# SysCV/LiDAR_snow_sim

Measured on AMD Instinct MI355X. Metric: augmented points/s/GPU (64x2048 sweep, 2.5 mm/h); HBM roofline % -- value: rows resident in HBM when the clock starts (device-resident API: augment_batch on CUDA tensors); with H2D of the rows and D2H of the results inside the clock: value_pcie_inclusive, higher is better.
Workload: dtype f64

## Files before the change

lidar_snow_sim_amd/csrc/sg_few.h:

```cpp
#pragma once
#include "sg_beam.h"

template <int N>
struct SgFew {
    double amp[N], rho[N];
    int k0[N], k1[N];
    double tamp, d;
    int tk0, tk1;
    int S;
};

template <typename T, int N>
__device__ __forceinline__ int sg_few_prep(double d, double theta_c, int L, const double (&a1_in)[N], const double (&a2_in)[N], const double (&rho)[N],
                                           int channel, const SgLasers *__restrict__ las, double beam_div_deg, SgFew<N> &p, SgBeamOut &out)
{
    constexpr bool F32 = SgReal<T>::is_f32;
    static_assert(N >= 1 && N <= 3, "an owner must stay below eight slots (2 N + 1 <= 7)");
    const int max_i = las->max_i[channel];
    double a1[N], a2[N];
    double theta_r, theta_l;
    sg_beam_limits(theta_c, beam_div_deg, theta_r, theta_l);
    double ra = theta_r, la = theta_l;
    const bool wrap = ra > la;
    if (wrap) ra = ra - SG_TWO_PI;
#pragma unroll
    for (int j = 0; j < N; ++j) {
        a1[j] = a1_in[j]; a2[j] = a2_in[j];
        if (wrap && j < L && a1[j] > a2[j]) a1[j] = a1[j] - SG_TWO_PI;
    }
    const double delta = beam_div_deg * (SG_PI / 180.0);
    double e_min = ra < la ? ra : la, e_max = ra < la ? la : ra;
#pragma unroll
    for (int j = 0; j < N; ++j) {
        if (j < L) {
            const double lo = a1[j], hi = a2[j];
            if (lo < e_min) e_min = lo;
            if (hi < e_min) e_min = hi;
            if (lo > e_max) e_max = lo;
            if (hi > e_max) e_max = hi;
        }
    }
    double R[N], tsum = -0.0;
    bool has[N];
#pragma unroll
    for (int j = 0; j < N; ++j) { R[j] = 0.0; has[j] = false; }
    for (double e = e_min; e < e_max;) {
        int own = -1;
        double nxt = e_max;
#pragma unroll
        for (int j = 0; j < N; ++j) {
            if (j < L) {
                if (own < 0 && a1[j] <= e && e < a2[j]) own = j;
                if (a1[j] > e && a1[j] < nxt) nxt = a1[j];
                if (a2[j] > e && a2[j] < nxt) nxt = a2[j];
            }
        }
        if (ra > e && ra < nxt) nxt = ra;
        if (la > e && la < nxt) nxt = la;
        const double w = nxt - e;
        if (own < 0) tsum += w;
#pragma unroll
        for (int j = 0; j < N; ++j)
            if (own == j) { R[j] = has[j] ? R[j] + w : w; has[j] = true; }
        e = nxt;
    }
    const double c_tau = 299792458.0 * 1e-8;
    const double beta_0 = 1 * 1e-6 / SG_PI;
    const double i_snow = 0.9 * max_i;
    const double ca_p0 = i_snow / beta_0;
#pragma unroll
    for (int t = 0; t < N; ++t) { p.amp[t] = 0.0; p.rho[t] = 0.0; p.k0[t] = 0; p.k1[t] = 0; }
    int S = 0;
#pragma unroll
    for (int j = 0; j < N; ++j) {
        if (j < L && has[j]) {
            const double ratio = sg_clip01((0.0 + R[j]) / delta);
            const double r = rho[j];
            int k0 = (int)ceil(r * 10);
            int k1 = (int)(floor((r + c_tau) * 10) + 1);
            const double amp = (((ca_p0 * beta_0) * ratio) * sg_xsi(r)) / (r * r);
            if (k1 > SG_RBINS) { out.range_error = 1; k1 = SG_RBINS; }
            if (k0 < 0) k0 = 0;
#pragma unroll
            for (int t = 0; t <= j; ++t)
                if (t == S) { p.amp[t] = amp; p.rho[t] = r; p.k0[t] = k0; p.k1[t] = k1; }
            ++S;
        }
    }
    p.S = S;
    p.d = d;
    p.tamp = 0.0; p.tk0 = 0; p.tk1 = 0;
    if (S == 0) return 0;
    const double ratio_t = sg_clip01((0.0 + tsum) / delta);
    if constexpr (F32) {
        const float r = (float)(T)d;
        p.tk0 = (int)ceilf(r * 10.0f);
        float ee = r + (float)c_tau;
        ee = ee * 10.0f;
        ee = floorf(ee) + 1.0f;
        p.tk1 = (int)ee;
        const float r2 = r * r;
        p.tamp = (((ca_p0 * beta_0) * ratio_t) * sg_xsi(r)) / (double)r2;
    } else {
        p.tk0 = (int)ceil(d * 10);
        p.tk1 = (int)(floor((d + c_tau) * 10) + 1);
        p.tamp = (((ca_p0 * beta_0) * ratio_t) * sg_xsi(d)) / (d * d);
    }
    if (p.tk1 > SG_RBINS) { out.range_error = 1; p.tk1 = SG_RBINS; }
    if (p.tk0 < 0) p.tk0 = 0;
    out.n_flakes = S;
    out.has_power = 1;
    return S;
}

template <int N, int TT>
__device__ __forceinline__ void sg_few_zone(const SgFew<N> &p, double best, int &ka, int &kb)
{
    constexpr bool TARGET = TT == N;
    const double c_tau = 299792458.0 * 1e-8;
    const double step = (120 + c_tau) / (SG_RBINS - 1);
    ka = 0; kb = -1;
    double A, r;
    int k0, k1;
    if constexpr (TARGET) { A = p.tamp; r = p.d; k0 = p.tk0; k1 = p.tk1; }
    else { if (TT >= p.S) return; A = p.amp[TT]; r = p.rho[TT]; k0 = p.k0[TT]; k1 = p.k1[TT]; }
    if (!(A > 0.0)) return;
    double oth = 0.0;
    int lo_trim = k0, hi_trim = k1;
    auto visit = [&](double Aj, int q0, int q1, bool first) {
        if (Aj > A || (Aj == A && first)) {
            if (q0 <= k0) { if (q1 > lo_trim) lo_trim = q1; }
            else if (q1 >= k1) { if (q0 < hi_trim) hi_trim = q0; }
        } else oth += Aj;
    };
    bool go = true;
#pragma unroll
    for (int j = N - 1; j >= 0; --j) {
        if (j < TT && j < p.S && go) {
            if (p.k1[j] <= k0) go = false;
            else visit(p.amp[j], p.k0[j], p.k1[j], true);
        }
    }
    if constexpr (!TARGET) {
        go = true;
#pragma unroll
        for (int j = 0; j < N; ++j) {
            if (j > TT && j < p.S && go) {
                if (p.k0[j] >= k1) go = false;
                else visit(p.amp[j], p.k0[j], p.k1[j], false);
            }
        }
        if (go && !(p.tk0 >= k1)) visit(p.tamp, p.tk0, p.tk1, false);
    }
    double amax = p.tamp;
#pragma unroll
    for (int j = 0; j < N; ++j) if (j < p.S) amax = fmax(amax, p.amp[j]);
    const double need = fmax(best, 0.9966 * amax);
    if ((A + oth) * (1.0 + 1e-9) < need) return;
    const double q = (need * (1.0 - 1e-9) - oth * (1.0 + 1e-9)) / A;
    ka = k0; kb = k1 - 1;
    if (q >= 0.5) {
        const double om = q < 1.0 ? 1.0 - q : 0.0;
        const double dl = (double)sqrtf((float)(1.26 * om)) * (1.0 + 1e-6) + 1e-6;
        const double Rc = r + c_tau / 2;
        const double D = dl * (c_tau / SG_PI) + 0.006;
        const int za = (int)ceil((Rc - D) * (1.0 / step)), zb = (int)floor((Rc + D) * (1.0 / step));
        if (za > ka) ka = za;
        if (zb < kb) kb = zb;
    }
    if (lo_trim > ka) ka = lo_trim;
    if (hi_trim - 1 < kb) kb = hi_trim - 1;
}

template <bool EXACT, int N>
__device__ __forceinline__ double sg_few_bin(const double (&amp)[N], const double (&rho)[N], const int (&k0)[N], const int (&k1)[N],
                                             double tamp, double d, int tk0, int tk1, int k, const double *__restrict__ rgrid)
{
    const double Rk = EXACT ? rgrid[k < SG_RBINS ? k : SG_RBINS - 1] : sg_range_bin(k);
    double sm = 0.0;
#pragma unroll
    for (int t = 0; t < N; ++t)
        if (k >= k0[t] && k < k1[t]) sm += sg_power_term<EXACT>(amp[t], Rk, rho[t]);
    if (k >= tk0 && k < tk1) sm += sg_power_term<EXACT>(tamp, Rk, d);
    return sm;
}
```

lidar_snow_sim_amd/csrc/snowgpu_kernels.hip:

```cpp
#include <hip/hip_runtime.h>
#include <algorithm>
#include "sg_beam.h"
#include "sg_few.h"
#include "sg_queue.h"
#include "sg_kutil.h"
#include "sg_launch.h"

#ifndef SG_NB4
#define SG_NB4 4
#endif
#ifndef SG_KP_WIN
#define SG_KP_WIN 3
#endif
#ifndef SG_FP_WAVES
#define SG_FP_WAVES 6
#endif
#ifndef SG_FP_WAVES_SEG
#define SG_FP_WAVES_SEG 7
#endif
#ifndef SG_NB_TIERS
#define SG_NB_TIERS 4
#endif
#ifndef SG_KP_THREE_MAX
#define SG_KP_THREE_MAX 16
// ... 390 lines not shown
        if ((threadIdx.x & 63) == 63 && total > 0) b = atomicAdd(counter, total);
        return __shfl(b, 63) + inc - n;
    };
    int base = reserve(n_items, a.pw_count);
    if (a.pw_items1) {
        int base1 = reserve(n_one, a.pw_count + 1);
        for (int k = 0; k < nf; k += lanes)
            a.pw_items1[base1++] = make_int2((int)(q_base + k), (nf - k < lanes ? nf - k : lanes) | (f1 << 10));
    } else {
        for (int k = 0; k < nf; k += lanes)
            a.pw_items[base++] = make_int2((int)(q_base + k), (nf - k < lanes ? nf - k : lanes) | (f1 << 10));
    }
    for (int k = 0; k < nb; k += lanes_back)
        a.pw_items[base++] = make_int2((int)(q_base + q_size - nb + k), (nb - k < lanes_back ? nb - k : lanes_back) | (f1 << 10));
}

__global__ __launch_bounds__(256) void k_tier_gather(SgBeamArgs a, int n_regions_ub)
{
    const int r = blockIdx.x * 4 + (int)(threadIdx.x >> 6), lane = (int)(threadIdx.x & 63);
    if (blockIdx.x == 0 && threadIdx.x < SG_MAX_CLASSES) a.status[2 + threadIdx.x] = a.tier_info[threadIdx.x];
    if (blockIdx.x == 0 && threadIdx.x < SG_MAX_CLASSES && a.tier_hint) a.tier_hint[threadIdx.x] = a.tier_info[threadIdx.x];
    if (blockIdx.x == 0 && threadIdx.x == 0 && a.tier_hint) a.tier_hint[SG_MAX_CLASSES] = (int32_t)((a.n_total >> 10) + 1);
    int q_size = 0, f1 = 0;
    int64_t q_base = 0;
    if (!sg_region(a, r, n_regions_ub, q_base, q_size, f1)) return;
    for (int k = 0; k < a.n_cls; ++k) {
        const int c = a.tn[(int64_t)r * SG_MAX_CLASSES + k];
        if (c == 0) continue;
        const int32_t *src = a.tier_sparse + (int64_t)k * a.tier_stride + q_base;
        int32_t *dst = a.tier_list + (int64_t)k * a.tier_stride + a.tbase[(int64_t)r * SG_MAX_CLASSES + k];
        for (int i = lane; i < c; i += 64) dst[i] = src[i];
    }
}

__device__ __forceinline__ const SgEntry *sg_dq_entries(const SgBeamArgs &a, int f, int ch)
{
    return a.frame_tables[(int64_t)f * a.las->n + ch].entries;
}

template <typename T, int LMAX, int BLOCK, bool LISTQ>
__device__ __forceinline__ void sg_kp_item(const SgBeamArgs &a, char *smem, const int ov_list, const int64_t work_off,
                                           const int start, const int cnt, const int item_f)
{
    constexpr int LANES = BLOCK < 64 ? BLOCK : 64;
    constexpr int WIN = BLOCK < 64 ? 1 : SG_KP_WIN;
    constexpr int P = SG_QPLANES(LMAX);
    double *s_a1 = (double *)smem;
    constexpr bool THREE = SG_KP_THREE_MAX > 0 && LMAX <= SG_KP_THREE_MAX && LMAX >= SG_KP_THREE_MIN;
    double *s_a2 = s_a1 + (LMAX + 1) * BLOCK;
    double *s_rho = s_a2 + (LMAX + 1) * BLOCK;
    double *s_ratio = THREE ? s_rho : s_rho + (LMAX + 1) * BLOCK;
    double *s_work = THREE ? s_a2 : s_ratio;
    const int tid = threadIdx.x, lane = tid & 63;
    const int ltid = BLOCK < 64 ? lane : tid;
    const double *planes = a.tq;
    const uint16_t *scs = LISTQ ? a.tq_sc : a.dq_sc;
    static_assert(WIN <= 4, "the window's permutation passes through one 64-double row segment of the wave");
    uint16_t *s_perm = (uint16_t *)(s_ratio + (BLOCK < 64 ? 0 : (tid & ~63)));
    int perm[WIN];
    const bool sorted = WIN > 1 && cnt > LANES;
    if constexpr (WIN > 1) {
        if (sorted) {
            int key[WIN], rank[WIN];
            int64_t at[WIN];
            unsigned scw[WIN];
#pragma unroll
            for (int r = 0; r < WIN; ++r) { const int idx = r * 64 + lane; at[r] = (int64_t)start + (idx < cnt ? idx : 0); }
            if (LISTQ && ov_list) {
#pragma unroll
                for (int r = 0; r < WIN; ++r) at[r] = (int64_t)a.tier_list[work_off + at[r]];
#pragma unroll
                for (int r = 0; r < WIN; ++r) scw[r] = (unsigned)a.ov_sc[at[r]];
            } else {
#pragma unroll
                for (int r = 0; r < WIN; ++r) scw[r] = (unsigned)scs[at[r]];
            }
#pragma unroll
            for (int r = 0; r < WIN; ++r) {
                const int idx = r * 64 + lane;
                key[r] = 255;
                if (idx < cnt) key[r] = scw[r] == 0xffffu ? 254 : (int)(scw[r] & 255u);
                rank[r] = 0;
            }
            int base = 0;
            auto place = [&](int c) {
#pragma unroll
                for (int r = 0; r < WIN; ++r) {
                    const unsigned long long m = __ballot(key[r] == c);
                    if (key[r] == c) rank[r] = base + (int)__popcll(m & sg_lanemask_lt());
                    base += (int)__popcll(m);
                }
            };
            for (int c = 0; c <= LMAX; ++c) place(c);
            place(254); place(255);
#pragma unroll
            for (int r = 0; r < WIN; ++r) s_perm[rank[r]] = (uint16_t)(r * 64 + lane);
            asm volatile("s_waitcnt lgkmcnt(0)" ::: "memory");
#pragma unroll
            for (int r = 0; r < WIN; ++r) perm[r] = s_perm[r * 64 + lane];
            asm volatile("s_waitcnt lgkmcnt(0)" ::: "memory");
        }
    }
    const int rounds = (cnt + LANES - 1) / LANES;
    for (int r = 0; r < rounds; ++r) {
        const int idx = r * LANES + lane;
        const bool in = lane < LANES && idx < cnt;
        int pos = idx;
        if constexpr (WIN > 1) {
            if (sorted) {
#pragma unroll
                for (int q = 0; q < WIN; ++q) if (q == r) pos = perm[q];
            }
        }
        const int64_t slot = (int64_t)start + pos;
        unsigned sc = 0xffffu;
        int32_t g = 0;
        double d = 0.0, tc = 0.0, f_rho = 0.0;
        [[maybe_unused]] double f_a1 = 0.0, f_a2 = 0.0;
        [[maybe_unused]] const double *qb = planes;
        [[maybe_unused]] int qs = 64;
        constexpr int NW = LMAX <= 4 ? LMAX : 1;
        [[maybe_unused]] uint32_t hw[NW];
#pragma unroll
        for (int j = 0; j < NW; ++j) hw[j] = 0u;
        if (in) {
            if constexpr (LISTQ) {
                g = a.tier_list[work_off + slot];
                if (ov_list) { qb = a.ov + (size_t)g * SG_OV_STRIDE; qs = 1; sc = a.ov_sc[g]; }
                else { qb = planes + sg_qaddr<P>(slot, 0); sc = scs[slot]; }
                d = qb[0];
                tc = qb[qs];
                f_a1 = qb[2 * qs]; f_a2 = qb[3 * qs]; f_rho = qb[4 * qs];
            } else {
                g = a.dq_g[slot];
                sc = scs[slot];
                sg_dq_load_header<T>(a.dq, slot, LMAX, d, tc);
#pragma unroll
                for (int j = 0; j < NW; ++j) hw[j] = sg_dq_load_word<T>(a.dq, slot, LMAX, j);
            }
        }
        const bool live = in && sc != 0xffffu;
        const int L = (int)(sc & 255u), ch = (int)(sc >> 8);
        int f = 0;
        SgBeamOut o;
        o.overflow = 0; o.range_error = 0; o.diff2 = 0.0; o.has_power = 0; o.n_flakes = 0; o.n_hits = 0; o.label = 0; o.new_i = 0; o.k_best = 0;
        constexpr int NB = LMAX <= 4 ? SG_NB4 : SG_NB_TIERS;
        int S = 0, nw = 0, k_best = 0;
        double best = 0.0;
        if (live) {
            f = item_f >= 0 ? item_f : sg_frame_of(a, g);
            unsigned long long ord = 0xfedcba9876543210ull;
            [[maybe_unused]] const SgEntry *ent = nullptr;
            if constexpr (LISTQ) {
                s_a1[ltid] = f_a1; s_a2[ltid] = f_a2; s_rho[ltid] = f_rho;
                if constexpr (THREE) ord = 0;
                for (int h0 = 1; h0 < L; h0 += 8) {
                    double xa[8], xb[8], xr[8];
#pragma unroll
                    for (int c = 0; c < 8; ++c) {
                        const int h = h0 + c < L ? h0 + c : 0;
                        xa[c] = qb[(2 + 3 * h) * qs]; xb[c] = qb[(3 + 3 * h) * qs]; xr[c] = qb[(4 + 3 * h) * qs];
                    }
#pragma unroll
                    for (int c = 0; c < 8; ++c)
                        if (h0 + c < L) { s_a1[(h0 + c) * BLOCK + ltid] = xa[c]; s_a2[(h0 + c) * BLOCK + ltid] = xb[c]; s_rho[(h0 + c) * BLOCK + ltid] = xr[c]; }
                }
                for (int h = 1; h < L; ++h) {
                    const double x1 = s_a1[h * BLOCK + ltid], x2 = s_a2[h * BLOCK + ltid], r = s_rho[h * BLOCK + ltid];
                    int q = h;
                    while (q > 0 && (s_rho[(q - 1) * BLOCK + ltid] > r ||
                                     (s_rho[(q - 1) * BLOCK + ltid] == r && ov_list &&
                                      (s_a1[(q - 1) * BLOCK + ltid] > x1 || (s_a1[(q - 1) * BLOCK + ltid] == x1 && s_a2[(q - 1) * BLOCK + ltid] > x2))))) {
                        s_rho[q * BLOCK + ltid] = s_rho[(q - 1) * BLOCK + ltid]; s_a1[q * BLOCK + ltid] = s_a1[(q - 1) * BLOCK + ltid];
                        s_a2[q * BLOCK + ltid] = s_a2[(q - 1) * BLOCK + ltid];
                        --q;
                    }
                    if (q != h) { s_rho[q * BLOCK + ltid] = r; s_a1[q * BLOCK + ltid] = x1; s_a2[q * BLOCK + ltid] = x2; }
                    if constexpr (THREE) {
                        const unsigned long long low = (1ull << (4 * q)) - 1ull;
                        ord = (ord & low) | ((unsigned long long)h << (4 * q)) | ((ord & ~low) << 4);
                    }
                }
            } else {
                ent = sg_dq_entries(a, f, ch);
                double th_r, th_l;
                sg_beam_limits(tc, a.beam_div_deg, th_r, th_l);
                if constexpr (LMAX <= 4) {
                    double xa[LMAX], xb[LMAX], xr[LMAX];
                    sg_dq_resolve_all<LMAX>(hw, L, ent, th_r, th_l, xa, xb, xr);
                    f_rho = xr[0];
#pragma unroll
                    for (int j = 0; j < LMAX; ++j)
                        if (j < L) {
                            s_a1[j * BLOCK + ltid] = xa[j]; s_a2[j * BLOCK + ltid] = xb[j];
                            if constexpr (!THREE) s_rho[j * BLOCK + ltid] = xr[j];
                        }
                } else {
                    for (int j0 = 0; j0 < L; j0 += 8) {
                        uint32_t w8[8];
                        double xa[8], xb[8], xr[8];
                        w8[0] = j0 == 0 ? hw[0] : sg_dq_load_word<T>(a.dq, slot, LMAX, j0);
#pragma unroll
                        for (int c = 1; c < 8; ++c) w8[c] = sg_dq_load_word<T>(a.dq, slot, LMAX, j0 + c < L ? j0 + c : 0);
                        sg_dq_resolve_all<8>(w8, L - j0, ent, th_r, th_l, xa, xb, xr);
                        if (j0 == 0) f_rho = xr[0];
#pragma unroll
                        for (int c = 0; c < 8; ++c)
                            if (j0 + c < L) {
                                s_a1[(j0 + c) * BLOCK + ltid] = xa[c]; s_a2[(j0 + c) * BLOCK + ltid] = xb[c];
                                if constexpr (!THREE) s_rho[(j0 + c) * BLOCK + ltid] = xr[c];
                            }
                    }
                }
            }
            auto queue_rho = [&](int j) -> double {
                const int h = (int)((ord >> (4 * j)) & 15ull);
                if constexpr (LISTQ) return h == 0 ? f_rho : qb[(4 + 3 * h) * qs];
                else return h == 0 ? f_rho : sg_dq_rho(sg_dq_load_word<T>(a.dq, slot, LMAX, h), ent);
            };
            int32_t *dc = a.dbg_count ? a.dbg_count + g : nullptr;
            double *drj = a.dbg_count ? a.dbg_rj + (int64_t)g * a.dbg_cap : nullptr;
            double *dra = a.dbg_count ? a.dbg_ratio + (int64_t)g * a.dbg_cap : nullptr;
            unsigned long long srcmap = 0;
            if constexpr (THREE) S = sg_beam_dict<LMAX, BLOCK, false>(L, tc, d, a.beam_div_deg, s_a1, s_a2, nullptr, s_ratio, ltid, 0, nullptr, nullptr, nullptr, 0, &srcmap);
            else S = sg_beam_dict<LMAX, BLOCK>(L, tc, d, a.beam_div_deg, s_a1, s_a2, s_rho, s_ratio, ltid, a.dbg_cap, dc, drj, dra);
            if constexpr (THREE) {
                if (dc) {
                    *dc = S + 1;
                    for (int t = 0; t <= S && t < a.dbg_cap; ++t) {
                        const int j = (int)((srcmap >> (4 * t)) & 15ull);
                        drj[t] = t == S ? d : queue_rho(j);
                        dra[t] = s_ratio[t * BLOCK + ltid];
                    }
                }
            }
            if (S > 0) {
                const T d_t = (T)d;
                if constexpr (THREE) {
                    sg_beam_amp3<T, LMAX, BLOCK>(d_t, S, ch, a.las, s_a1, s_a2, s_rho, ltid, o,
                                                 [&](int t) { return queue_rho((int)((srcmap >> (4 * t)) & 15ull)); });
                } else sg_beam_amp<T, LMAX, BLOCK>(d_t, S, ch, a.las, s_a1, s_a2, s_rho, s_ratio, ltid, o, 0);
                if (o.range_error) {
                    atomicCAS(&a.status[0], 0, 4 );
                    atomicCAS(&a.status[1], -1, g);
                }
                if (a.exact_math) nw = sg_power_plan<BLOCK, true, NB, LMAX>(S, a.rgrid, s_a1, s_a2, s_rho, s_work, ltid, best, k_best);
                else nw = sg_power_plan<BLOCK, false, NB, LMAX>(S, a.rgrid, s_a1, s_a2, s_rho, s_work, ltid, best, k_best);
            } else S = 0;
        }
        {
            const int colbase = BLOCK < 64 ? 0 : (tid & ~63);
            if (a.exact_math) sg_wave_eval<BLOCK, true, NB>(nw, S, a.rgrid, s_a1, s_a2, s_rho, s_work, colbase, best, k_best);
            else sg_wave_eval<BLOCK, false, NB>(nw, S, a.rgrid, s_a1, s_a2, s_rho, s_work, colbase, best, k_best);
        }
        if (live) {
            uint32_t rec = 0;
            if (S > 0) {
                sg_beam_decide(d, ch, a.las, best, k_best, o);
                rec = sg_pack_record(o);
            }
            if (LISTQ) a.rec[g] = rec;
            else a.rec_q[slot] = rec;
        }
        sg_add_diff2(a.diff2, live, f, live ? (long long)o.diff2 : 0);
    }
}

template <typename T, int LMAX, int BLOCK, bool LISTQ>
__global__ __launch_bounds__(BLOCK < 64 ? 64 : BLOCK, LMAX <= 4 ? SG_KP_WAVES : (LMAX <= 16 ? SG_KP_WAVES_TIERS : 1)) void k_power(SgBeamArgs a)
{
    constexpr int THREADS = BLOCK < 64 ? 64 : BLOCK, WAVES = THREADS / 64, LANES = BLOCK < 64 ? BLOCK : 64;
    constexpr int WIN = BLOCK < 64 ? 1 : SG_KP_WIN;
    extern __shared__ __attribute__((aligned(16))) char smem[];
    if constexpr (LMAX > 16) __builtin_amdgcn_s_setprio(3);
    const int tid = threadIdx.x;
    int64_t work_n = 0, work_off = 0;
    int n_items;
    const int step = (int)gridDim.x * WAVES;
    int item_slots = LANES * WIN;
    if (LISTQ) {
        work_n = a.tier_info[a.cls];
        if (work_n > a.work_hi) work_n = a.work_hi;
        work_off = (int64_t)a.cls * a.tier_stride;
        if (WIN > 1 && work_n <= (int64_t)step * LANES) item_slots = LANES;
        n_items = (int)((work_n + item_slots - 1) / item_slots);
    } else {
        n_items = *a.pw_count;
    }
    for (int i = (int)blockIdx.x * WAVES + __builtin_amdgcn_readfirstlane(tid >> 6); i < n_items; i += step) {
        int start, cnt, item_f = -1;
        if (LISTQ) {
            start = i * item_slots;
            cnt = (int)(work_n - start < item_slots ? work_n - start : item_slots);
        } else {
            const int2 d = a.pw_items[i];
            start = __builtin_amdgcn_readfirstlane(d.x);
            const int dy = __builtin_amdgcn_readfirstlane(d.y);
            cnt = dy & 1023; item_f = (dy >> 10) - 1;
        }
        sg_kp_item<T, LMAX, BLOCK, LISTQ>(a, smem, a.ov_list, work_off, start, cnt, item_f);
    }
}

template <typename T, int N>
__global__ __launch_bounds__(256, 4) void k_power_few(SgBeamArgs a, int lmax)
{
    __shared__ double s_amp[N + 1][256], s_rho[N + 1][256], s_best[256];
    __shared__ int s_win[N + 1][256], s_zone[N + 1][256], s_k[256];
    __shared__ int s_mark[256];
    const int tid = (int)threadIdx.x, lane = tid & 63, wbase = tid & ~63;
    const int n_items = a.pw_count[1];
    const int step = (int)gridDim.x * 4;
    for (int i = (int)blockIdx.x * 4 + __builtin_amdgcn_readfirstlane(tid >> 6); i < n_items; i += step) {
        const int2 it = a.pw_items1[i];
        const int start = __builtin_amdgcn_readfirstlane(it.x), dy = __builtin_amdgcn_readfirstlane(it.y);
        const int cnt = dy & 1023, item_f = (dy >> 10) - 1;
        const bool live = lane < cnt;
        const int64_t slot = (int64_t)start + lane;
        SgBeamOut o;
        o.overflow = 0; o.range_error = 0; o.diff2 = 0.0; o.has_power = 0; o.n_flakes = 0; o.n_hits = 0; o.label = 0; o.new_i = 0; o.k_best = 0;
        int f = 0, ch = 0, S = 0, g = 0;
        SgFew<N> P{};
        int zone[N + 1], n = 0;
#pragma unroll
        for (int z = 0; z <= N; ++z) zone[z] = 0;
        if (live) {
            const unsigned sc = a.dq_sc[slot];
            double d, tc;
            sg_dq_load_header<T>(a.dq, slot, lmax, d, tc);
            uint32_t w[N];
#pragma unroll
            for (int j = 0; j < N; ++j) w[j] = sg_dq_load_word<T>(a.dq, slot, lmax, j);
            ch = (int)(sc >> 8);
            g = a.dq_g[slot];
            f = item_f >= 0 ? item_f : sg_frame_of(a, g);
            const SgEntry *ent = sg_dq_entries(a, f, ch);
            double th_r, th_l, a1[N], a2[N], rho[N];
            sg_beam_limits(tc, a.beam_div_deg, th_r, th_l);
            sg_dq_resolve_all<N>(w, (int)(sc & 255u), ent, th_r, th_l, a1, a2, rho);
            S = sg_few_prep<T, N>(d, tc, (int)(sc & 255u), a1, a2, rho, ch, a.las, a.beam_div_deg, P, o);
            if (S) {
                int ka, kb;
                sg_few_zone<N, 0>(P, 0.0, ka, kb);
                if (kb >= ka) { zone[0] = ka | ((kb - ka + 1) << 16); n += kb - ka + 1; }
                if constexpr (N >= 2) { sg_few_zone<N, 1>(P, 0.0, ka, kb); if (kb >= ka) { zone[1] = ka | ((kb - ka + 1) << 16); n += kb - ka + 1; } }
                if constexpr (N >= 3) { sg_few_zone<N, 2>(P, 0.0, ka, kb); if (kb >= ka) { zone[2] = ka | ((kb - ka + 1) << 16); n += kb - ka + 1; } }
                sg_few_zone<N, N>(P, 0.0, ka, kb);
                if (kb >= ka) { zone[N] = ka | ((kb - ka + 1) << 16); n += kb - ka + 1; }
            }
        }
#pragma unroll
        for (int t = 0; t < N; ++t) { s_amp[t][tid] = P.amp[t]; s_rho[t][tid] = P.rho[t]; s_win[t][tid] = P.k0[t] | (P.k1[t] << 16); }
        s_amp[N][tid] = P.tamp; s_rho[N][tid] = P.d; s_win[N][tid] = P.tk0 | (P.tk1 << 16);
#pragma unroll
        for (int z = 0; z <= N; ++z) s_zone[z][tid] = zone[z];
        s_best[tid] = 0.0; s_k[tid] = 0;
        asm volatile("" ::: "memory");
        const int incl = sg_wave_incl_add(n);
        const int excl = incl - n;
        const int total = __builtin_amdgcn_readlane(incl, 63);
        for (int base = 0; base < total; base += 64) {
            const int p = base + lane;
            const bool valid = p < total;
#if !defined(SG_FEW_OWNER_SEARCH)
            const int ow = sg_pair_owner(s_mark, tid, base, excl, incl);
#else
            int lo = 0, hi = 63;
            for (int s6 = 0; s6 < 6; ++s6) {
                const int mid = (lo + hi) >> 1;
                const int v = __shfl(incl, mid);
                if (v > p) hi = mid; else lo = mid + 1;
            }
            const int ow = lo & 63;
#endif
            int j = p - __shfl(excl, ow);
            double sm = -1.0;
            int kk = 0x7fffffff, oo = 64 + lane;
            if (valid) {
                const int col = wbase + ow;
                int k = 0;
                bool found = false;
#pragma unroll
                for (int z = 0; z <= N; ++z) {
                    const int zc = s_zone[z][col], zn = (int)((unsigned)zc >> 16);
                    if (!found) { if (j < zn) { k = (zc & 0xffff) + j; found = true; } else j -= zn; }
                }
                double amp[N], rho[N];
                int k0[N], k1[N];
#pragma unroll
                for (int t = 0; t < N; ++t) {
                    amp[t] = s_amp[t][col]; rho[t] = s_rho[t][col];
                    const int w = s_win[t][col];
                    k0[t] = w & 0xffff; k1[t] = (int)((unsigned)w >> 16);
                }
                const int tw = s_win[N][col];
                sm = a.exact_math ? sg_few_bin<true, N>(amp, rho, k0, k1, s_amp[N][col], s_rho[N][col], tw & 0xffff, (int)((unsigned)tw >> 16), k, a.rgrid)
                                  : sg_few_bin<false, N>(amp, rho, k0, k1, s_amp[N][col], s_rho[N][col], tw & 0xffff, (int)((unsigned)tw >> 16), k, a.rgrid);
                kk = k; oo = ow;
            }
            sg_fold_runs(sm, kk, oo);
            const int on = sg_dpp<0x130, 0xf>(oo, oo);
            if (valid && (lane == 63 || on != oo)) {
                volatile double *vb = s_best;
                volatile int *vk = s_k;
                const int col = wbase + oo;
                const double b0 = vb[col];
                const int kc = vk[col];
                if (sm > b0 || (sm == b0 && kk < kc)) { vb[col] = sm; vk[col] = kk; }
            }
        }
        asm volatile("s_waitcnt lgkmcnt(0)" ::: "memory");
        if (live) {
            uint32_t rec = 0;
            if (S) {
                const double best = ((volatile double *)s_best)[tid];
                const int k_best = ((volatile int *)s_k)[tid];
                if (o.range_error) {
                    atomicCAS(&a.status[0], 0, 4 );
                    atomicCAS(&a.status[1], -1, g);
                }
                sg_beam_decide(P.d, ch, a.las, best, k_best, o);
                rec = sg_pack_record(o);
            }
            a.rec_q[slot] = rec;
        }
        sg_add_diff2(a.diff2, live, f, live ? (long long)o.diff2 : 0);
        asm volatile("s_waitcnt lgkmcnt(0)" ::: "memory");
    }
}

template <typename T>
__global__ __launch_bounds__(64) void k_beams_huge(SgBeamArgs a)
{
    const int tid = (int)(blockIdx.x * 64 + threadIdx.x);
    const int rstride = a.h_lanes;
    const size_t col = (size_t)(a.h_cap + 1) * (size_t)a.h_lanes;
    double *s_a1 = a.h_lists, *s_a2 = s_a1 + col, *s_rho = s_a2 + col, *s_ratio = s_rho + col;
    const int n_las = a.las->n;
    int64_t work_n = a.tier_info[a.cls];
    const int64_t work_off = (int64_t)a.cls * a.tier_stride;
    int64_t chunk = (int64_t)blockIdx.x * 64;
    if (chunk >= work_n) return;
    do {
    const bool live = chunk + threadIdx.x < work_n;
    int64_t g = 0;
    int f = 0;
    SgBeamOut o;
    o.overflow = 0; o.range_error = 0; o.diff2 = 0.0; o.has_power = 0; o.n_flakes = 0; o.n_hits = 0; o.label = 0; o.new_i = 0; o.k_best = 0;
    if (live) {
        g = a.tier_list[work_off + chunk + threadIdx.x];
        f = sg_frame_of(a, g);
        const T *row = sg_row<T>(a, f, g);
        const T px = row[0], py = row[1], pz = row[2];
        const int ch = (int)row[4];
        const SgTable tab = a.frame_tables[(int64_t)f * n_las + ch];
        int32_t *dc = a.dbg_count ? a.dbg_count + g : nullptr;
        double *drj = a.dbg_count ? a.dbg_rj + g * a.dbg_cap : nullptr;
        double *dra = a.dbg_count ? a.dbg_ratio + g * a.dbg_cap : nullptr;
        sg_beam<T, 0, 0>(px, py, pz, ch, tab, a.las, a.beam_div_deg, s_a1, s_a2, s_rho, s_ratio, tid, o, a.dbg_cap, dc, drj,
                                dra, a.exact_math != 0, rstride, a.h_cap);
        uint32_t rec = 0;
        if (o.overflow) {
            atomicCAS(&a.status[0], 0, 6 );
            atomicCAS(&a.status[1], -1, (int32_t)g);
        } else if (o.range_error) {
            atomicCAS(&a.status[0], 0, 4 );
            atomicCAS(&a.status[1], -1, (int32_t)g);
        }
        if (o.has_power) {
            double best = 0.0;
            int k_best = 0;
            if (a.exact_math) sg_lane_power<0, true, 8, 0>(o.n_flakes, a.rgrid, s_a1, s_a2, s_rho, s_ratio, tid, best, k_best, rstride, a.h_cap);
            else sg_lane_power<0, false, 8, 0>(o.n_flakes, a.rgrid, s_a1, s_a2, s_rho, s_ratio, tid, best, k_best, rstride, a.h_cap);
            T d_t;
            if constexpr (SgReal<T>::is_f32) d_t = sqrtf((px * px + py * py) + pz * pz);
            else d_t = sqrt((px * px + py * py) + pz * pz);
            sg_beam_decide((double)d_t, ch, a.las, best, k_best, o);
            rec = sg_pack_record(o);
        }
        a.rec[g] = rec;
    }
    sg_add_diff2(a.diff2, live, f, live ? (long long)o.diff2 : 0);
    } while ((chunk += (int64_t)gridDim.x * 64) < work_n);
}


template <typename T, int LMAX, int BLOCK, bool LIST, int DICT, bool SEG = false>
static int launch_beams_t(const SgBeamArgs *a, hipStream_t st)
{
    const size_t lds = DICT ? (sizeof(double) + sizeof(uint32_t)) * (size_t)BLOCK * (size_t)LMAX
                                  + sizeof(int) * (3 * (size_t)(BLOCK < 64 ? 64 : BLOCK) + (size_t)LMAX * BLOCK)
                            : sizeof(double) * (size_t)BLOCK * 4 * ((size_t)LMAX + 1);
    static bool attr_set[64] = {};
    if (int e = sg_set_lds(k_beams<T, LMAX, BLOCK, LIST, DICT, SEG>, lds, attr_set)) return e;
    constexpr int THREADS = BLOCK < 64 ? 64 : BLOCK;
    unsigned blocks;
    if (LIST) {
        const int64_t n = (int64_t)a->work_hi - a->work_lo;
        if (n <= 0) return 0;
        const unsigned per_cu = (unsigned)std::min<size_t>(32 * 64 / THREADS, std::max<size_t>(1, (size_t)(160 * 1024) / lds));
        blocks = (unsigned)std::min<int64_t>((n + BLOCK - 1) / BLOCK, (int64_t)sg_cu_count() * per_cu);
        blocks = std::min(blocks, 128u);
    } else {
        blocks = (unsigned)a->grid_blocks;
    }
    if (blocks == 0) return 0;
    hipLaunchKernelGGL((k_beams<T, LMAX, BLOCK, LIST, DICT, SEG>), dim3(blocks), dim3(THREADS), lds, st, *a);
    SG_CHECK_LAUNCH();
    return 0;
}

template <typename T, int LMAX, int BLOCK, bool LISTQ>
static int launch_power_t(const SgBeamArgs *a, hipStream_t st, bool plan_only = false, hipEvent_t ev_few = nullptr, int which = 3)
{
    const size_t lds = sizeof(double) * ((size_t)BLOCK * ((SG_KP_THREE_MAX > 0 && LMAX <= SG_KP_THREE_MAX && LMAX >= SG_KP_THREE_MIN) ? 3 : 4) * (LMAX + 1));
    static bool attr_set[64] = {};
    if (int e = sg_set_lds(k_power<T, LMAX, BLOCK, LISTQ>, lds, attr_set)) return e;
    constexpr int THREADS = BLOCK < 64 ? 64 : BLOCK, LANES = BLOCK < 64 ? BLOCK : 64;
    const int cus = sg_cu_count();
    unsigned per_cu = (unsigned)std::min<size_t>(32 * 64 / THREADS, std::max<size_t>(1, (size_t)(160 * 1024) / lds));
    if (!LISTQ && a->kp_lds_quarters > 0 && a->kp_lds_quarters < 4) per_cu = std::max(1u, per_cu * (unsigned)a->kp_lds_quarters / 4u);
    int64_t blocks = (int64_t)cus * per_cu;
    int64_t items_ub = LISTQ ? ((int64_t)a->work_hi + LANES - 1) / LANES : (a->n_total + LANES - 1) / LANES + 2 * a->n_regions_ub;
    if (LISTQ && a->work_hint > 0) items_ub = std::min<int64_t>(items_ub, (4 * (int64_t)a->work_hint + LANES - 1) / LANES + 8);
    blocks = std::min<int64_t>(blocks, (items_ub + THREADS / 64 - 1) / (THREADS / 64));
    if (blocks <= 0) return 0;
    if (!LISTQ) {
        const unsigned pg = (unsigned)((a->n_regions_ub + 255) / 256);
        if (pg == 0) return 0;
        const int64_t back_est = a->n_total / 10;
        const int lanes_back = (BLOCK < 64 || back_est <= (int64_t)blocks * (THREADS / 64) * LANES * 5 / 2) ? LANES : LANES * SG_KP_WIN;
        if (plan_only) {
            hipLaunchKernelGGL(k_power_plan, dim3(pg), dim3(256), 0, st, *a, LANES, lanes_back, (int)a->n_regions_ub);
            SG_CHECK_LAUNCH();
            return 0;
        }
        if (a->pw_items1 && (which & 1)) {
            hipStream_t s1 = st;
            const unsigned g1 = (unsigned)std::min<int64_t>((int64_t)cus * 4, (a->n_total / LANES + a->n_regions_ub + 3) / 4);
            if (g1 > 0) {
                if (a->front_max == 1) hipLaunchKernelGGL((k_power_few<T, 1>), dim3(g1), dim3(256), 0, s1, *a, LMAX);
                else if (a->front_max == 2) hipLaunchKernelGGL((k_power_few<T, 2>), dim3(g1), dim3(256), 0, s1, *a, LMAX);
                else hipLaunchKernelGGL((k_power_few<T, 3>), dim3(g1), dim3(256), 0, s1, *a, LMAX);
            }
            SG_CHECK_LAUNCH();
            if (ev_few && hipEventRecord(ev_few, st) != hipSuccess) return (int)hipGetLastError();
        }
    }
    if (!(which & 2)) return 0;
    hipLaunchKernelGGL((k_power<T, LMAX, BLOCK, LISTQ>), dim3((unsigned)blocks), dim3(THREADS), lds, st, *a);
    SG_CHECK_LAUNCH();
    return 0;
}

extern "C" int sg_launch_tier_scan(const SgBeamArgs *a, int dtype, int lmax, void *stream)
{
    const int64_t n = (int64_t)a->work_hi - a->work_lo;
    if (n <= 0) return 0;
    int64_t want = (n + 255) / 256;
    if (a->work_hint > 0) want = std::min<int64_t>(want, (4 * (int64_t)a->work_hint + 255) / 256 + 8);
    const unsigned blocks = (unsigned)std::min<int64_t>(want, (int64_t)sg_cu_count() * 8);
    return sg_by_dtype_tier<false>(dtype, lmax, [&](auto t, auto tier) {
        hipLaunchKernelGGL((k_tier_scan_direct<decltype(t), decltype(tier)::LMAX>), dim3(blocks), dim3(256), 0, (hipStream_t)stream, *a);
        SG_CHECK_LAUNCH();
        return 0;
    });
}

extern "C" int sg_beams_block(int lmax)
{
    return sg_by_tier<true>(lmax, [](auto tier) { return decltype(tier)::BLOCK; });
}

extern "C" int sg_launch_beams(const SgBeamArgs *a, int dtype, int lmax, int direct, void *stream)
{
    hipStream_t st = (hipStream_t)stream;
    return sg_by_dtype_tier<true>(dtype, lmax, [&](auto t, auto tier) {
        using T = decltype(t);
        constexpr int LMAX = decltype(tier)::LMAX, BLOCK = decltype(tier)::BLOCK;
        if (!direct) return launch_beams_t<T, LMAX, BLOCK, true, 0>(a, st);
        if (a->exact_math) return a->seg_blk ? launch_beams_t<T, LMAX, BLOCK, false, 2, true>(a, st)
                                             : launch_beams_t<T, LMAX, BLOCK, false, 2>(a, st);
        return a->seg_blk ? launch_beams_t<T, LMAX, BLOCK, false, 1, true>(a, st) : launch_beams_t<T, LMAX, BLOCK, false, 1>(a, st);
    });
}

extern "C" int sg_launch_power(const SgBeamArgs *a, int dtype, int lmax, void *stream, int plan_only, void *ev_few, int which)
{
    return sg_by_dtype_tier<true>(dtype, lmax, [&](auto t, auto tier) {
        return launch_power_t<decltype(t), decltype(tier)::LMAX, decltype(tier)::BLOCK, false>(a, (hipStream_t)stream, plan_only != 0, (hipEvent_t)ev_few, which);
    });
}

extern "C" int sg_launch_tier_gather(const SgBeamArgs *a, void *stream)
{
    const unsigned g = (unsigned)((a->n_regions_ub + 3) / 4);
    if (g == 0) return 0;
    hipLaunchKernelGGL(k_tier_gather, dim3(g), dim3(256), 0, (hipStream_t)stream, *a, (int)a->n_regions_ub);
    SG_CHECK_LAUNCH();
    return 0;
}

extern "C" int sg_launch_power_list(const SgBeamArgs *a, int dtype, int lmax, void *stream)
{
    return sg_by_dtype_tier<false>(dtype, lmax, [&](auto t, auto tier) {
        return launch_power_t<decltype(t), decltype(tier)::LMAX, decltype(tier)::BLOCK, true>(a, (hipStream_t)stream);
    });
}

extern "C" int sg_launch_huge(const SgBeamArgs *a, int dtype, void *stream)
{
    const unsigned blocks = (unsigned)(a->h_lanes / 64);
    if (blocks == 0) return 0;
    return sg_by_dtype(dtype, [&](auto t) {
        hipLaunchKernelGGL(k_beams_huge<decltype(t)>, dim3(blocks), dim3(64), 0, (hipStream_t)stream, *a);
        SG_CHECK_LAUNCH();
        return 0;
    });
}
```

Baseline: 10.33 billion.

## Route LMAX=4 back-pass power items through the few-flake kernel

Extends the few-flake power kernel to N=4 by adding an exact-summation fallback when an owner accumulates eight or more angular slots. Items in the back list for the LMAX=4, 256-thread tier then go to k_power_few<T,4,2,true> instead of the general LDS-heavy k_power, and the planner keeps those items at single-wave granularity. The goal is to replace the general per-bin power loop with the cheaper zone-pruned path for beams with up to four flakes. The cost is higher register and LDS pressure, occupancy bounded at two waves per SIMD, and a possible second slot-walk pass.

After: 10.54 billion (median of 6 runs). +2.0%, better.

```diff
diff --git a/lidar_snow_sim_amd/csrc/sg_few.h b/lidar_snow_sim_amd/csrc/sg_few.h
--- a/lidar_snow_sim_amd/csrc/sg_few.h
+++ b/lidar_snow_sim_amd/csrc/sg_few.h
@@ -15,7 +15,8 @@
                                            int channel, const SgLasers *__restrict__ las, double beam_div_deg, SgFew<N> &p, SgBeamOut &out)
 {
     constexpr bool F32 = SgReal<T>::is_f32;
-    static_assert(N >= 1 && N <= 3, "an owner must stay below eight slots (2 N + 1 <= 7)");
+    static_assert(N >= 1 && N <= 4, "2 N + 1 <= 9 slots: four bits count an owner's, and one block of eight addends is all SgNpSum sees");
+    constexpr bool COUNT = 2 * N + 1 >= 8;
     const int max_i = las->max_i[channel];
     double a1[N], a2[N];
     double theta_r, theta_l;
@@ -42,10 +43,11 @@
     }
     double R[N], tsum = -0.0;
     bool has[N];
+    [[maybe_unused]] unsigned cnt = 0;
 #pragma unroll
     for (int j = 0; j < N; ++j) { R[j] = 0.0; has[j] = false; }
-    for (double e = e_min; e < e_max;) {
-        int own = -1;
+    auto slot_at = [&](double e, int &own) -> double {
+        own = -1;
         double nxt = e_max;
 #pragma unroll
         for (int j = 0; j < N; ++j) {
@@ -57,12 +59,37 @@
         }
         if (ra > e && ra < nxt) nxt = ra;
         if (la > e && la < nxt) nxt = la;
+        return nxt;
+    };
+    for (double e = e_min; e < e_max;) {
+        int own;
+        const double nxt = slot_at(e, own);
         const double w = nxt - e;
         if (own < 0) tsum += w;
 #pragma unroll
         for (int j = 0; j < N; ++j)
             if (own == j) { R[j] = has[j] ? R[j] + w : w; has[j] = true; }
+        if constexpr (COUNT) cnt += 1u << (4 * (own < 0 ? N : own));
         e = nxt;
+    }
+    if constexpr (COUNT) {
+        if (cnt & (0x88888888u >> (28 - 4 * N))) {
+#pragma unroll
+            for (int t = 0; t <= N; ++t) {
+                if (((cnt >> (4 * t)) & 15u) < 8u) continue;
+                SgNpSum acc;
+                acc.reset();
+                for (double e = e_min; e < e_max;) {
+                    int own;
+                    const double nxt = slot_at(e, own);
+                    if ((own < 0 ? N : own) == t) acc.push(nxt - e);
+                    e = nxt;
+                }
+                if (t == N) tsum = acc.result();
+#pragma unroll
+                for (int j = 0; j < N; ++j) if (j == t) R[j] = acc.result();
+            }
+        }
     }
     const double c_tau = 299792458.0 * 1e-8;
     const double beta_0 = 1 * 1e-6 / SG_PI;
diff --git a/lidar_snow_sim_amd/csrc/snowgpu_kernels.hip b/lidar_snow_sim_amd/csrc/snowgpu_kernels.hip
--- a/lidar_snow_sim_amd/csrc/snowgpu_kernels.hip
+++ b/lidar_snow_sim_amd/csrc/snowgpu_kernels.hip
@@ -716,17 +716,18 @@
     }
 }
 
-template <typename T, int N>
-__global__ __launch_bounds__(256, 4) void k_power_few(SgBeamArgs a, int lmax)
+template <typename T, int N, int WPS = 4, bool BACK = false>
+__global__ __launch_bounds__(256, WPS) void k_power_few(SgBeamArgs a, int lmax)
 {
     __shared__ double s_amp[N + 1][256], s_rho[N + 1][256], s_best[256];
     __shared__ int s_win[N + 1][256], s_zone[N + 1][256], s_k[256];
     __shared__ int s_mark[256];
     const int tid = (int)threadIdx.x, lane = tid & 63, wbase = tid & ~63;
-    const int n_items = a.pw_count[1];
+    const int n_items = a.pw_count[BACK ? 0 : 1];
+    const int2 *__restrict__ items = BACK ? a.pw_items : a.pw_items1;
     const int step = (int)gridDim.x * 4;
     for (int i = (int)blockIdx.x * 4 + __builtin_amdgcn_readfirstlane(tid >> 6); i < n_items; i += step) {
-        const int2 it = a.pw_items1[i];
+        const int2 it = items[i];
         const int start = __builtin_amdgcn_readfirstlane(it.x), dy = __builtin_amdgcn_readfirstlane(it.y);
         const int cnt = dy & 1023, item_f = (dy >> 10) - 1;
         const bool live = lane < cnt;
@@ -759,6 +760,7 @@
                 if (kb >= ka) { zone[0] = ka | ((kb - ka + 1) << 16); n += kb - ka + 1; }
                 if constexpr (N >= 2) { sg_few_zone<N, 1>(P, 0.0, ka, kb); if (kb >= ka) { zone[1] = ka | ((kb - ka + 1) << 16); n += kb - ka + 1; } }
                 if constexpr (N >= 3) { sg_few_zone<N, 2>(P, 0.0, ka, kb); if (kb >= ka) { zone[2] = ka | ((kb - ka + 1) << 16); n += kb - ka + 1; } }
+                if constexpr (N >= 4) { sg_few_zone<N, 3>(P, 0.0, ka, kb); if (kb >= ka) { zone[3] = ka | ((kb - ka + 1) << 16); n += kb - ka + 1; } }
                 sg_few_zone<N, N>(P, 0.0, ka, kb);
                 if (kb >= ka) { zone[N] = ka | ((kb - ka + 1) << 16); n += kb - ka + 1; }
             }
@@ -931,6 +933,8 @@
     static bool attr_set[64] = {};
     if (int e = sg_set_lds(k_power<T, LMAX, BLOCK, LISTQ>, lds, attr_set)) return e;
     constexpr int THREADS = BLOCK < 64 ? 64 : BLOCK, LANES = BLOCK < 64 ? BLOCK : 64;
+    constexpr bool BACK_FEW = !LISTQ && LMAX == 4 && BLOCK == 256;
+    const bool back_few = BACK_FEW && a->pw_items1;
     const int cus = sg_cu_count();
     unsigned per_cu = (unsigned)std::min<size_t>(32 * 64 / THREADS, std::max<size_t>(1, (size_t)(160 * 1024) / lds));
     if (!LISTQ && a->kp_lds_quarters > 0 && a->kp_lds_quarters < 4) per_cu = std::max(1u, per_cu * (unsigned)a->kp_lds_quarters / 4u);
@@ -943,7 +947,7 @@
         const unsigned pg = (unsigned)((a->n_regions_ub + 255) / 256);
         if (pg == 0) return 0;
         const int64_t back_est = a->n_total / 10;
-        const int lanes_back = (BLOCK < 64 || back_est <= (int64_t)blocks * (THREADS / 64) * LANES * 5 / 2) ? LANES : LANES * SG_KP_WIN;
+        const int lanes_back = (BLOCK < 64 || back_few || back_est <= (int64_t)blocks * (THREADS / 64) * LANES * 5 / 2) ? LANES : LANES * SG_KP_WIN;
         if (plan_only) {
             hipLaunchKernelGGL(k_power_plan, dim3(pg), dim3(256), 0, st, *a, LANES, lanes_back, (int)a->n_regions_ub);
             SG_CHECK_LAUNCH();
@@ -962,6 +966,14 @@
         }
     }
     if (!(which & 2)) return 0;
+    if constexpr (BACK_FEW) {
+        if (back_few) {
+            const unsigned g4 = (unsigned)std::min<int64_t>((int64_t)cus * 2, (a->n_total / LANES + a->n_regions_ub + 3) / 4);
+            if (g4 > 0) hipLaunchKernelGGL((k_power_few<T, 4, 2, true>), dim3(g4), dim3(256), 0, st, *a, LMAX);
+            SG_CHECK_LAUNCH();
+            return 0;
+        }
+    }
     hipLaunchKernelGGL((k_power<T, LMAX, BLOCK, LISTQ>), dim3((unsigned)blocks), dim3(THREADS), lds, st, *a);
     SG_CHECK_LAUNCH();
     return 0;
```
